# nrclaudio/spVIPES

Hardware: AMD Instinct MI355X
Metric: cells/sec/training-step (2-group PoE VAE) (higher is better)
Workload: dtype bf16

## Files before the change

### spvipes_amd/csrc/spv_abi.hip

```cpp
#include "../../include/spvipes_hip.h"
#include "spv_common.h"
#include "spv_gemm.h"
#include "spv_fc1.h"
#include "spv_dec_gemm.h"
#include "spv_decoder.h"
#include "spv_dec_expected.h"
#include "spv_dec_sample.h"
#include "spv_dec_sample_stats.h"
#include "spv_dec_expected_stats.h"
#include "spv_de.h"
#include "spv_de_median.h"
#include "spv_count_stats.h"
#include "spv_knn.h"
#include "spv_ot.h"
#include "spv_silhouette.h"
#include "spv_small.h"
#include "spv_poe_n.h"

#include <cstdio>
#include <cstdlib>
#include <cstring>

using namespace spv;

// ... 1721 lines not shown
  return SPV_OK;
}
extern "C" int spv_poe_comp_fwd(const spv_poe_comp_args* a, void* stream) {
  int rc = check_poe_comp(a, "spv_poe_comp_fwd", false);
  if (rc) return rc;
  hipStream_t s = (hipStream_t)stream;
  int Bm = 0;
  for (int g = 0; g < a->ngroups; ++g) Bm = a->B[g] > Bm ? a->B[g] : Bm;
  const int W = 2 * a->n + 1;
  hipLaunchKernelGGL(pn_stats_kernel, dim3(PN_SEG, a->ngroups), dim3(128), 0, s, *a);
  hipLaunchKernelGGL(pn_means_kernel, dim3((a->ncomp * W + 255) / 256, a->ngroups), dim3(256), 0, s, *a);
  hipLaunchKernelGGL(pn_fuse_fwd_kernel, dim3((Bm + 7) / 8, a->ngroups), dim3(256), 0, s, *a);
  return launch_status("spv_poe_comp_fwd");
}
extern "C" int spv_poe_comp_bwd(const spv_poe_comp_args* a, void* stream) {
  int rc = check_poe_comp(a, "spv_poe_comp_bwd", true);
  if (rc) return rc;
  hipStream_t s = (hipStream_t)stream;
  int Bm = 0;
  for (int g = 0; g < a->ngroups; ++g) Bm = a->B[g] > Bm ? a->B[g] : Bm;
  hipLaunchKernelGGL(pn_cell_bwd_kernel, dim3((Bm + 7) / 8, a->ngroups), dim3(256), 0, s, *a);
  hipLaunchKernelGGL(pn_comp_bwd_kernel, dim3(PN_SEG, a->ngroups), dim3(64), 0, s, *a);
  hipLaunchKernelGGL(pn_apply_bwd_kernel, dim3((Bm + 7) / 8, a->ngroups), dim3(256), 0, s, *a);
  return launch_status("spv_poe_comp_bwd");
}

extern "C" int spv_zsplit_fwd(const spv_zsplit_args* a, void* stream) {
  if (!a || a->B <= 0 || a->n_p <= 0 || a->n_s <= 0 || a->ngroups <= 0 || a->ngroups > 2) return fail(SPV_ERR_ARG, "spv_zsplit_fwd: bad shape%s");
  for (int g = 0; g < a->ngroups; ++g) if (!a->priv[g] || !a->poe[g] || !a->zcat[g]) return fail(SPV_ERR_ARG, "spv_zsplit_fwd: null pointer%s");
  const long tot = (long)a->B * (a->n_p + a->n_s);
  bool pack = false, pack_all = true;
  for (int g = 0; g < a->ngroups; ++g) { pack = pack || a->am_hi[g] || a->aps_hi[g]; pack_all = pack_all && a->am_hi[g] && a->aps_hi[g]; }
  if (!pack_all) hipLaunchKernelGGL(zsplit_fwd_kernel, dim3((unsigned)((tot + 255) / 256), a->ngroups), dim3(256), 0, (hipStream_t)stream, *a);
  if (pack) {
    const int kp = a->kslots ? SPV_DEC_KP_WIDE : SPV_DEC_KP, ks = a->kslots ? SPV_DEC_KS_WIDE : SPV_DEC_KS;
    if (a->Bp < a->B || (a->kslots != 0 && a->kslots != 1) || a->n_p + 1 > kp || a->n_s + 1 > ks || a->am_cols < a->n_p + a->n_s + 1 || a->am_cols < 0 ||
        a->ld_am < a->am_col + a->am_cols)
      return fail(SPV_ERR_ARG, "spv_zsplit_fwd: bad operand-image shape%s");
    const long tp = (long)a->Bp * (kp + ks + a->am_cols);
    if (a->kslots) hipLaunchKernelGGL(zsplit_pack_kernel<2>, dim3((unsigned)((tp + 255) / 256), a->ngroups), dim3(256), 0, (hipStream_t)stream, *a);
    else hipLaunchKernelGGL(zsplit_pack_kernel<1>, dim3((unsigned)((tp + 255) / 256), a->ngroups), dim3(256), 0, (hipStream_t)stream, *a);
  }
  return launch_status("spv_zsplit_fwd");
}
extern "C" int spv_zsplit_bwd(const spv_zsplit_args* a, void* stream) {
  if (!a || a->B <= 0 || a->n_p <= 0 || a->n_s <= 0 || a->ngroups <= 0 || a->ngroups > 2) return fail(SPV_ERR_ARG, "spv_zsplit_bwd: bad shape%s");
  for (int g = 0; g < a->ngroups; ++g) if (!a->d_zcat[g] || !a->d_priv[g] || !a->d_poe[g]) return fail(SPV_ERR_ARG, "spv_zsplit_bwd: null pointer%s");
  const long tot = (long)a->B * (a->n_p + a->n_s);
  hipLaunchKernelGGL(zsplit_bwd_kernel, dim3((unsigned)((tot + 255) / 256), a->ngroups), dim3(256), 0, (hipStream_t)stream, *a);
  return launch_status("spv_zsplit_bwd");
}

static int check_fold(const spv_fold_batch* a, const char* who) {
  if (!a || a->nprob <= 0 || a->nprob > SPV_MAXP || a->B <= 0) return fail(SPV_ERR_ARG, "%s: bad batch", who);
  if (a->kslots != 0 && a->kslots != 1) return fail(SPV_ERR_ARG, "%s: kslots must be 0 or 1", who);
  const int kmax = a->kslots ? FOLD_KMAX_WIDE : FOLD_KMAX;
  for (int i = 0; i < a->nprob; ++i) {
    const spv_fold_prob& q = a->p[i];
    if (q.K <= 0 || q.K > kmax || q.G <= 0 || q.Gp < q.G || !q.W || !q.gamma || !q.beta || !q.running_mean || !q.running_var || !q.stat ||
        (a->training && (!q.zsum || !q.zz)))
      return fail(SPV_ERR_ARG, "%s: bad problem (K <= 32, or 64 with kslots = 1; non-null pointers)", who);
  }
  return SPV_OK;
}
extern "C" int spv_bn_fold_fwd(const spv_fold_batch* a, void* stream) {
  int rc = check_fold(a, "spv_bn_fold_fwd");
  if (rc) return rc;
  int gmax = 0;
  for (int i = 0; i < a->nprob; ++i) {
    const spv_fold_prob& q = a->p[i];
    if (!q.img_hi || !q.img_lo || q.slot < q.K + 1 || q.col_off + q.slot > q.ld_img) return fail(SPV_ERR_ARG, "spv_bn_fold_fwd: bad image slot%s");
    if ((q.slot | q.col_off | q.ld_img) % 8 || ((reinterpret_cast<uintptr_t>(q.img_hi) | reinterpret_cast<uintptr_t>(q.img_lo)) & 15))
      return fail(SPV_ERR_ARG, "spv_bn_fold_fwd: slot, col_off, ld_img must be multiples of 8 elements and the images 16-byte aligned%s");
    gmax = q.Gp > gmax ? q.Gp : gmax;
  }
  if (a->kslots) hipLaunchKernelGGL(bn_fold_fwd_kernel<FOLD_KMAX_WIDE>, dim3((gmax + FOLD_FWD_GENES - 1) / FOLD_FWD_GENES, a->nprob), dim3(256), 0, (hipStream_t)stream, *a);
  else hipLaunchKernelGGL(bn_fold_fwd_kernel<FOLD_KMAX>, dim3((gmax + FOLD_FWD_GENES - 1) / FOLD_FWD_GENES, a->nprob), dim3(256), 0, (hipStream_t)stream, *a);
  return launch_status("spv_bn_fold_fwd");
}
extern "C" int spv_bn_fold_bwd(const spv_fold_batch* a, void* stream) {
  int rc = check_fold(a, "spv_bn_fold_bwd");
  if (rc) return rc;
  int gmax = 0;
  for (int i = 0; i < a->nprob; ++i) {
    const spv_fold_prob& q = a->p[i];
    if (!q.dWeff || !q.dW || !q.dgamma || !q.dbeta || q.ld_dw < q.K + 1 || (a->training && (!q.red_part || !q.z || !q.dz)))
      return fail(SPV_ERR_ARG, "spv_bn_fold_bwd: null pointer%s");
    gmax = q.G > gmax ? q.G : gmax;
  }
  hipStream_t s = (hipStream_t)stream;
  if (a->kslots) hipLaunchKernelGGL(bn_fold_bwd_kernel<FOLD_KMAX_WIDE>, dim3((gmax + 255) / 256, a->nprob), dim3(FOLD_BWD_THREADS), 0, s, *a);
  else hipLaunchKernelGGL(bn_fold_bwd_kernel<FOLD_KMAX>, dim3((gmax + 255) / 256, a->nprob), dim3(FOLD_BWD_THREADS), 0, s, *a);
  if (a->training) {
    for (int i = 0; i < a->nprob; ++i) {
      const spv_fold_prob& q = a->p[i];
      if (q.out_priv && (!q.out_poe || q.n_p <= 0 || q.n_s <= 0 || q.zcol < 0 || q.zcol + q.K > q.n_p + q.n_s))
        return fail(SPV_ERR_ARG, "spv_bn_fold_bwd: bad latent-slicing outputs%s");
    }
    if (a->kslots) hipLaunchKernelGGL(zstats_bwd_kernel<FOLD_KMAX_WIDE>, dim3((a->B + 63) / 64, a->nprob), dim3(256), 0, s, *a);
    else hipLaunchKernelGGL(zstats_bwd_kernel<FOLD_KMAX>, dim3((a->B + 63) / 64, a->nprob), dim3(256), 0, s, *a);
  }
  return launch_status("spv_bn_fold_bwd");
}

static int check_trunk(const spv_trunk_batch* a, const char* who) {
  if (!a || a->nprob <= 0 || a->nprob > 2 || a->B <= 0) return fail(SPV_ERR_ARG, "%s: bad batch", who);
  for (int i = 0; i < a->nprob; ++i) {
    const spv_trunk_prob& q = a->p[i];
    if (q.N <= 0 || q.N > 256 || q.K <= 0 || q.K > SPV_TRUNK_KMAX) return fail(SPV_ERR_UNSUPPORTED, "%s: N <= 256 and K <= 48", who);
    if (!q.W || !q.gamma || !q.beta || !q.running_mean || !q.running_var || !q.stat) return fail(SPV_ERR_ARG, "%s: null pointer", who);
    if (a->training && (!q.zsum || !q.zz)) return fail(SPV_ERR_ARG, "%s: training mode needs the z statistics", who);
  }
  return SPV_OK;
}
extern "C" int spv_trunk_fold_fwd(const spv_trunk_batch* a, void* stream) {
  int rc = check_trunk(a, "spv_trunk_fold_fwd");
  if (rc) return rc;
  int nmax = 0;
  for (int i = 0; i < a->nprob; ++i) {
    if (!a->p[i].Wf || !a->p[i].cf) return fail(SPV_ERR_ARG, "spv_trunk_fold_fwd: null output%s");
    nmax = a->p[i].N > nmax ? a->p[i].N : nmax;
  }
  hipLaunchKernelGGL(trunk_fold_fwd_kernel, dim3((nmax + TRUNK_FWD_ROWS - 1) / TRUNK_FWD_ROWS, a->nprob), dim3(1024), 0, (hipStream_t)stream, *a);
  return launch_status("spv_trunk_fold_fwd");
}
extern "C" int spv_trunk_fold_bwd(const spv_trunk_batch* a, void* stream) {
  int rc = check_trunk(a, "spv_trunk_fold_bwd");
  if (rc) return rc;
  for (int i = 0; i < a->nprob; ++i) {
    const spv_trunk_prob& q = a->p[i];
    if (!q.dWf || !q.dcf || !q.dW || !q.dgamma || !q.dbeta) return fail(SPV_ERR_ARG, "spv_trunk_fold_bwd: null pointer%s");
    if (a->training && (!q.dred || !q.z || !q.dz || q.ldz < q.K || q.lddz < q.K)) return fail(SPV_ERR_ARG, "spv_trunk_fold_bwd: z-statistics buffers missing%s");
  }
  hipStream_t s = (hipStream_t)stream;
  int nmax = 0;
  for (int i = 0; i < a->nprob; ++i) nmax = a->p[i].N > nmax ? a->p[i].N : nmax;
  const int nblk = (nmax + TRUNK_BWD_ROWS - 1) / TRUNK_BWD_ROWS;
  hipLaunchKernelGGL(trunk_fold_bwd_kernel, dim3(nblk, a->nprob), dim3(1024), 0, s, *a);
  if (a->training) hipLaunchKernelGGL(trunk_zstats_kernel, dim3((a->B + 63) / 64, a->nprob), dim3(256), 0, s, *a, nblk);
  return launch_status("spv_trunk_fold_bwd");
}

extern "C" int spv_reduce_slabs(const spv_reduce_batch* b, void* stream) {
  if (!b || b->nprob <= 0 || b->nprob > SPV_MAXR) return fail(SPV_ERR_ARG, "spv_reduce_slabs: bad batch%s");
  long blocks = 1;
  for (int i = 0; i < b->nprob; ++i) {
    const spv_reduce_prob& q = b->p[i];
    if (!q.src || !q.dst || q.nslabs <= 0 || q.rows <= 0 || q.cols <= 0 || q.ld_src < q.col_off + q.cols || q.ld_dst < q.cols || q.col_off < 0 ||
        (long)q.rows * q.cols >= (1l << 31))
      return fail(SPV_ERR_ARG, "spv_reduce_slabs: bad problem%s");
    const long t = reduce_blocks_needed(q);
    if (t > blocks) blocks = t;
  }
  if (blocks > 8192) blocks = 8192;
  hipLaunchKernelGGL(reduce_slabs_kernel, dim3((unsigned)blocks, b->nprob), dim3(256), 0, (hipStream_t)stream, *b);
  return launch_status("spv_reduce_slabs");
}

extern "C" int spv_loss_assemble(const float* rec0, const float* rec1, const float* w, const float* const* kl, int32_t nkl, int32_t B,
                                 const float* kl_weight, float* loss, float* rec_sum, float* gkl, void* stream) {
  if (!rec0 || !w || !loss || B <= 0 || nkl < 0 || nkl > 4 || (nkl > 0 && !kl)) return fail(SPV_ERR_ARG, "spv_loss_assemble: bad arguments%s");
  const float* k[4] = {nullptr, nullptr, nullptr, nullptr};
  for (int i = 0; i < nkl; ++i) k[i] = kl[i];
  hipLaunchKernelGGL(loss_assemble_kernel, dim3(1), dim3(1024), 0, (hipStream_t)stream, rec0, rec1, w, k[0], k[1], k[2], k[3], B, kl_weight,
                     loss, rec_sum, gkl);
  return launch_status("spv_loss_assemble");
}

struct Fc1PrepArgs { const float* dh1; const float* h1; int B, N1; bf16_t* img_hi; bf16_t* img_lo; long ld_img; float* part; int nblk; float* db; float* db2; int n_first;
                     float* scale_ws; };

__device__ __forceinline__ float block_max_256(float v, float* s_red) {
#pragma unroll
  for (int off = 32; off > 0; off >>= 1) v = fmaxf(v, __shfl_xor(v, off, 64));
  if ((threadIdx.x & 63) == 0) s_red[threadIdx.x >> 6] = v;
  __syncthreads();
  return fmaxf(fmaxf(s_red[0], s_red[1]), fmaxf(s_red[2], s_red[3]));
}

__device__ __forceinline__ void fc1_bwd_prep_body(const Fc1PrepArgs& a, const int blk, float* s_red) {
  const int r0 = blk * 16;
  const bool half = a.img_lo == nullptr;
  float amax = 0.f;
  for (int col = threadIdx.x; col < (int)a.ld_img; col += 256) {
    float sum = 0.f;
#pragma unroll 4
    for (int r = r0; r < r0 + 16; ++r) {
      const long i = (long)min(r, a.B - 1) * a.N1 + min(col, a.N1 - 1);
      const float hv = a.h1[i], gv = a.dh1[i];
      const float v = (r < a.B && col < a.N1 && hv > 0.f) ? gv : 0.f;
      if (!half) {
        bf16_t hi, lo;
        split_bf16(v, hi, lo);
        a.img_hi[(long)r * a.ld_img + col] = hi;
        a.img_lo[(long)r * a.ld_img + col] = lo;
      }
      amax = fmaxf(amax, fabsf(v));
      sum += v;
    }
    if (col < a.N1) a.part[(long)blk * a.N1 + col] = sum;
  }
  if (half) {
    amax = block_max_256(amax, s_red);
    if (threadIdx.x == 0) a.scale_ws[2 + blk] = amax;
  }
}

__device__ __forceinline__ void fc1_bwd_finish_body(const Fc1PrepArgs& a, const int blk, float* s_red, float (*s_p)[64]) {
  const bool half = a.img_lo == nullptr;
  if (half && blk < a.nblk) {
    float m = 0.f;
    for (int k = threadIdx.x; k < a.nblk; k += 256) m = fmaxf(m, a.scale_ws[2 + k]);
    m = block_max_256(m, s_red);
    float scale, inv;
    pow2_scale_for(m, scale, inv);
    if (blk == 0 && threadIdx.x == 0) { a.scale_ws[0] = scale; a.scale_ws[1] = inv; }
    const int r0 = blk * 16;
    for (int col = threadIdx.x; col < (int)a.ld_img; col += 256) {
#pragma unroll 4
      for (int r = r0; r < r0 + 16; ++r) {
        const long i = (long)min(r, a.B - 1) * a.N1 + min(col, a.N1 - 1);
        const float hv = a.h1[i], gv = a.dh1[i];
        const float v = (r < a.B && col < a.N1 && hv > 0.f) ? gv : 0.f;
        a.img_hi[(long)r * a.ld_img + col] = f2h(v * scale);
      }
    }
  }
  if (blk >= (a.N1 + 63) / 64) return;
  const int tx = threadIdx.x & 63, ty = threadIdx.x >> 6;
  const int col = blk * 64 + tx;
  float v = 0.f;
  if (col < a.N1)
#pragma unroll 8
    for (int k = ty; k < a.nblk; k += 4) v += a.part[(long)k * a.N1 + col];
  s_p[ty][tx] = v;
  __syncthreads();
  if (ty != 0 || col >= a.N1) return;
  v = ((s_p[0][tx] + s_p[1][tx]) + s_p[2][tx]) + s_p[3][tx];
  if (a.db2 != nullptr && col >= a.n_first) a.db2[col - a.n_first] = v;
  else a.db[col] = v;
}

__global__ __launch_bounds__(256) void fc1_bwd_prep_kernel(Fc1PrepArgs a) {
  __shared__ float s_red[4];
  fc1_bwd_prep_body(a, blockIdx.x, s_red);
}
__global__ __launch_bounds__(256) void fc1_bwd_finish_kernel(Fc1PrepArgs a) {
  __shared__ float s_red[4];
  __shared__ float s_p[4][64];
  fc1_bwd_finish_body(a, blockIdx.x, s_red, s_p);
}
__global__ __launch_bounds__(256) void fc1_bwd_prep_pair_kernel(Fc1PrepArgs a0, Fc1PrepArgs a1) {
  __shared__ float s_red[4];
  const Fc1PrepArgs a = blockIdx.y ? a1 : a0;
  if ((int)blockIdx.x >= a.nblk) return;
  fc1_bwd_prep_body(a, blockIdx.x, s_red);
}
__global__ __launch_bounds__(256) void fc1_bwd_finish_pair_kernel(Fc1PrepArgs a0, Fc1PrepArgs a1) {
  __shared__ float s_red[4];
  __shared__ float s_p[4][64];
  const Fc1PrepArgs a = blockIdx.y ? a1 : a0;
  fc1_bwd_finish_body(a, blockIdx.x, s_red, s_p);
}
static int fc1_finish_blocks(const Fc1PrepArgs& a) {
  const int nb_bias = (a.N1 + 63) / 64;
  return (a.img_lo == nullptr && a.nblk > nb_bias) ? a.nblk : nb_bias;
}
static Fc1PrepArgs fc1_prep_args(const float* dh1, const float* h1, int B, int N1, uint16_t* img_hi, uint16_t* img_lo, long ld_img, int Bp, float* part, float* db,
                                 float* db2, int n_first, float* scale_ws) {
  return Fc1PrepArgs{dh1, h1, B, N1, (bf16_t*)img_hi, (bf16_t*)img_lo, ld_img, part, Bp / 16, db, db2, n_first, scale_ws};
}
static Fc1PrepArgs fc1_prep_args(const spv_fc1_bwd_args& a) {
  return fc1_prep_args(a.dh1, a.h1, a.B, a.N1, a.dh_hi, nullptr, a.ld_dh, a.Bp, a.part, a.db, a.db2, a.n_first, a.scale_ws);
}
static void fc1_prep_pair_launch(const spv_fc1_bwd_args& a, const spv_fc1_bwd_args& b, hipStream_t s) {
  const Fc1PrepArgs q0 = fc1_prep_args(a), q1 = fc1_prep_args(b);
  hipLaunchKernelGGL(fc1_bwd_prep_pair_kernel, dim3(max2(q0.nblk, q1.nblk), 2), dim3(256), 0, s, q0, q1);
  hipLaunchKernelGGL(fc1_bwd_finish_pair_kernel, dim3(max2(fc1_finish_blocks(q0), fc1_finish_blocks(q1)), 2), dim3(256), 0, s, q0, q1);
}

extern "C" int spv_enc_fc1_bwd_prep(const float* dh1, const float* h1, int32_t B, int32_t N1, uint16_t* img_hi, uint16_t* img_lo,
                                    int64_t ld_img, int32_t Bp, float* part, float* db, float* db2, int32_t n_first, float* scale_ws, void* stream) {
  if (!dh1 || !h1 || !img_hi || !part || !db) return fail(SPV_ERR_ARG, "spv_enc_fc1_bwd_prep: null pointer%s");
  if (B <= 0 || N1 <= 0 || Bp < B || (Bp % 64) || ld_img < N1) return fail(SPV_ERR_ARG, "spv_enc_fc1_bwd_prep: bad shape (Bp a multiple of 64)%s");
  if (!img_lo && !scale_ws) return fail(SPV_ERR_ARG, "spv_enc_fc1_bwd_prep: the f16 image (img_lo == NULL) needs scale_ws [2 + Bp / 16]%s");
  if (Bp / 16 > 65536) return fail(SPV_ERR_ARG, "spv_enc_fc1_bwd_prep: minibatch too large%s");
  hipStream_t s = (hipStream_t)stream;
  const Fc1PrepArgs a = fc1_prep_args(dh1, h1, B, N1, img_hi, img_lo, ld_img, Bp, part, db, db2, n_first, scale_ws);
  hipLaunchKernelGGL(fc1_bwd_prep_kernel, dim3(a.nblk), dim3(256), 0, s, a);
  hipLaunchKernelGGL(fc1_bwd_finish_kernel, dim3(fc1_finish_blocks(a)), dim3(256), 0, s, a);
  return launch_status("spv_enc_fc1_bwd_prep");
}

static bool fc1_fwd_dma_ok(const spv_fc1_fwd_args& a) {
  return a.x && a.x->X && a.W1_hi && a.bias && a.slabs && a.h1 && a.library && a.xb_all && a.library_all && a.B > 0 && a.G > 0 && a.splits > 0 &&
         spv_enc_fc1_fwd_uses_dma(a.B, a.G, a.N1, a.nsplit, 1, a.ldw, a.ld_xb) && aligned16(a.xb_all, a.W1_hi) &&
         (a.nsplit == 1 || (a.W1_lo && aligned16(a.W1_lo)));
}
static GemmParams fc1_fwd_dma_params(const spv_fc1_fwd_args& a) {
  GemmParams p{};
  p.A = a.xb_all; p.lda = a.ld_xb; p.B = a.W1_hi; p.ldb = a.ldw; p.rows = a.x->rows;
  if (a.nsplit == 3) p.B_lo = a.W1_lo;
  p.n_cells = a.B; p.n_genes = a.G; p.C = a.slabs; p.ldc = a.N1; p.M = a.B; p.N = a.N1; p.K = a.G;
  const int kt = (a.G + F1_BK - 1) / F1_BK;
  p.k_per_split = ((kt + a.splits - 1) / a.splits) * F1_BK;
  p.c_split_row = a.splits;
  return p;
// ... 364 lines not shown
```

### spvipes_amd/csrc/spv_small.h

```cpp
#pragma once
#include "../../include/spvipes_hip.h"
#include "spv_common.h"

namespace spv {


typedef spv_linear_prob LinearProb;
typedef spv_linear_batch LinearBatch;

__device__ __forceinline__ unsigned hash_u32(unsigned long long x) {
  x ^= x >> 33; x *= 0xff51afd7ed558ccdULL; x ^= x >> 33; x *= 0xc4ceb9fe1a85ec53ULL; x ^= x >> 33;
  return (unsigned)x;
}
__device__ __forceinline__ bool dropout_keep(unsigned long long seed, int prob, long idx, float p) {
  const unsigned key = ((unsigned)seed ^ ((unsigned)(seed >> 32) * 0x9E3779B9u)) + (unsigned)(prob + 1) * 0x85EBCA6Bu;
  unsigned x = (unsigned)idx * 747796405u + key;
  x = ((x >> ((x >> 28) + 4u)) ^ x) * 277803737u;
  x ^= x >> 22;
  x = x * 0x2C1B3C6Du + key;
  x ^= x >> 15;
  return (float)(x >> 8) * (1.0f / 16777216.0f) >= p;
}

__device__ __forceinline__ f16v mfma_f32(float x, float w, const f16v& c) { return __builtin_amdgcn_mfma_f32_32x32x2f32(x, w, c, 0, 0, 0); }
// ... 1332 lines not shown

constexpr int TRUNK_FWD_ROWS = 16;
__device__ __forceinline__ float trunk_Cw(const float* s_C, const float* wrow, int K, int l) {
  float t = 0.f;
  const int lc = min(l, K - 1);
#pragma unroll 4
  for (int k = 0; k < K; ++k) t += wrow[k] * s_C[k * K + lc];
  return (l < K) ? t : 0.f;
}
__global__ __launch_bounds__(1024) void trunk_fold_fwd_kernel(TrunkBatch a) {
  const TrunkProb& q = a.p[blockIdx.y];
  __shared__ float s_zbar[TRUNK_KMAX], s_C[TRUNK_KMAX * TRUNK_KMAX], s_wr[TRUNK_FWD_ROWS][64];
  const int K = q.K;
  if (blockIdx.x * TRUNK_FWD_ROWS >= q.N) return;
  const int l = threadIdx.x & 63, wv = threadIdx.x >> 6, j = blockIdx.x * TRUNK_FWD_ROWS + wv;
  const int ji = min(j, q.N - 1);
  const float wl = (l < K) ? q.W[(long)ji * K + l] : 0.f;
  const float bj = q.bias ? q.bias[ji] : 0.f;
  s_wr[wv][l] = wl;
  if (a.training) trunk_stats_to_lds(q, a.B, s_zbar, s_C, 1024);
  __syncthreads();
  if (j >= q.N) return;
  float mean0, var;
  if (a.training) {
    const float t = trunk_Cw(s_C, s_wr[wv], K, l);
    mean0 = wave_sum_all(wl * ((l < K) ? s_zbar[l] : 0.f));
    var = fmaxf(wave_sum_all(wl * t), 0.f);
    if (l == 0) {
      q.running_mean[j] = (1.f - a.momentum) * q.running_mean[j] + a.momentum * (mean0 + bj);
      q.running_var[j] = (1.f - a.momentum) * q.running_var[j] + a.momentum * var * ((float)a.B / fmaxf((float)a.B - 1.f, 1.f));
    }
  } else {
    mean0 = q.running_mean[j] - bj;
    var = q.running_var[j];
  }
  const float inv = q.gamma[j] * rsqrtf(var + a.eps);
  if (l < K) q.Wf[(long)j * K + l] = wl * inv;
  if (l == 0) { q.cf[j] = q.beta[j] - inv * mean0; q.stat[2 * j] = mean0; q.stat[2 * j + 1] = var; }
}

constexpr int TRUNK_BWD_ROWS = 64;
__global__ __launch_bounds__(1024) void trunk_fold_bwd_kernel(TrunkBatch a) {
  const TrunkProb& q = a.p[blockIdx.y];
  __shared__ float s_zbar[TRUNK_KMAX], s_C[TRUNK_KMAX * TRUNK_KMAX], s_w[TRUNK_BWD_ROWS * TRUNK_KMAX], s_dm[TRUNK_BWD_ROWS], s_dv[TRUNK_BWD_ROWS];
  const int K = q.K;
  const int j0 = blockIdx.x * TRUNK_BWD_ROWS;
  if (j0 >= q.N) return;
  if (a.training) trunk_stats_to_lds(q, a.B, s_zbar, s_C, 1024);
  __syncthreads();
  const int l = threadIdx.x & 63, wv = threadIdx.x >> 6;
  for (int pass = 0; pass < TRUNK_BWD_ROWS / 16; ++pass) {
    const int jl = 16 * pass + wv, j = j0 + jl;
    const bool real = j < q.N;
    const int ji = min(j, q.N - 1);
    const float wl = (real && l < K) ? q.W[(long)ji * K + l] : 0.f;
    const float gWl = (real && l < K) ? q.dWf[(long)ji * K + l] : 0.f;
    const float mean0 = q.stat[2 * ji], var = q.stat[2 * ji + 1];
    const float rs = rsqrtf(var + a.eps), gam = q.gamma[ji], inv = gam * rs;
    const float gc = real ? q.dcf[ji] : 0.f;
    const float dinv = wave_sum_all(gWl * wl) - gc * mean0;
    float dmean = 0.f, dvar = 0.f;
    if (real && l == 0) {
      q.dbeta[j] = gc;
      q.dgamma[j] = dinv * rs;
      if (q.dbias) q.dbias[j] = a.training ? 0.f : gc * inv;
    }
    if (a.training) {
      if (l < TRUNK_KMAX) s_w[jl * TRUNK_KMAX + l] = wl;
      const float v = trunk_Cw(s_C, s_w + jl * TRUNK_KMAX, K, l);
      if (real) { dmean = -gc * inv; dvar = dinv * gam * (-0.5f) * rs * rs * rs; }
      if (real && l < K) q.dW[(long)j * K + l] = gWl * inv + dmean * s_zbar[l] + 2.0f * dvar * v;
      if (l == 0) { s_dm[jl] = dmean; s_dv[jl] = dvar; }
    } else if (real && l < K) {
      q.dW[(long)j * K + l] = gWl * inv;
    }
  }
  if (!a.training) return;
  __syncthreads();
  const int lane = l, h = lane >> 5, r = lane & 31;
  if (wv >= 4) return;
  const int tr = wv >> 1, tc = wv & 1;
  if (32 * tr >= K || 32 * tc >= K) return;
  f16v accC, accM;
#pragma unroll
  for (int i = 0; i < 16; ++i) { accC[i] = 0.f; accM[i] = 0.f; }
  const int ca = 32 * tr + r, cb = 32 * tc + r;
  for (int t = 0; t < TRUNK_BWD_ROWS; t += 2) {
    const float wa = (ca < TRUNK_KMAX) ? s_w[(t + h) * TRUNK_KMAX + min(ca, TRUNK_KMAX - 1)] : 0.f;
    const float wb = (cb < TRUNK_KMAX) ? s_w[(t + h) * TRUNK_KMAX + min(cb, TRUNK_KMAX - 1)] : 0.f;
    accC = mfma_f32(s_dv[t + h] * wa, wb, accC);
    if (tr == 0) accM = mfma_f32((r == 0) ? s_dm[t + h] : 0.f, wb, accM);
  }
  float* out = q.dred + (long)blockIdx.x * (K + K * K);
#pragma unroll
  for (int i = 0; i < 16; ++i) {
    const int row = 32 * tr + crow(i, h), col = cb;
    if (row < K && col < K) out[K + row * K + col] = accC[i];
  }
  if (tr == 0 && h == 0 && cb < K) out[cb] = accM[0];
}

constexpr int TRUNK_ZS_KK = (TRUNK_KMAX + 3) / 4;
__global__ __launch_bounds__(256) void trunk_zstats_kernel(TrunkBatch a, int nblk) {
  const TrunkProb& q = a.p[blockIdx.y];
  __shared__ float s_zbar[TRUNK_KMAX], s_dz[TRUNK_KMAX], s_S[TRUNK_KMAX * TRUNK_KMAX], s_z[64 * (TRUNK_KMAX + 1)];
  const int K = q.K, nred = K + K * K;
  const float invB = 1.0f / (float)a.B;
  const int nb = (q.N + TRUNK_BWD_ROWS - 1) / TRUNK_BWD_ROWS;
  auto part4 = [&](int i) {
    float v[4];
#pragma unroll
    for (int u = 0; u < 4; ++u) v[u] = q.dred[(long)min(u, nb - 1) * nred + i];
    float d = v[0];
#pragma unroll
    for (int u = 1; u < 4; ++u) d += (u < nb) ? v[u] : 0.f;
    return d;
  };
  for (int i = threadIdx.x; i < K; i += 256) { s_zbar[i] = q.zsum[i] * invB; s_dz[i] = part4(i) * invB; }
  for (int i = threadIdx.x; i < K * K; i += 256) {
    const int k = i / K, l = i - k * K;
    s_S[i] = (part4(K + i) + part4(K + l * K + k)) * invB;
  }
  const int b0 = blockIdx.x * 64;
  __syncthreads();
  for (int i = threadIdx.x; i < 64 * K; i += 256) {
    const int c = i / K, l = i % K, b = min(b0 + c, a.B - 1);
    s_z[c * (TRUNK_KMAX + 1) + l] = q.z[(long)b * q.ldz + l] - s_zbar[l];
  }
  __syncthreads();
  const int c = threadIdx.x & 63, kg = threadIdx.x >> 6;
  float acc[TRUNK_ZS_KK];
#pragma unroll
  for (int kk = 0; kk < TRUNK_ZS_KK; ++kk) acc[kk] = s_dz[min(kg + 4 * kk, K - 1)];
  for (int l = 0; l < K; ++l) {
    const float zl = s_z[c * (TRUNK_KMAX + 1) + l];
#pragma unroll
    for (int kk = 0; kk < TRUNK_ZS_KK; ++kk) acc[kk] += s_S[min(kg + 4 * kk, K - 1) * K + l] * zl;
  }
  __syncthreads();
#pragma unroll
  for (int kk = 0; kk < TRUNK_ZS_KK; ++kk) {
    const int k = kg + 4 * kk;
    if (k < K) s_z[c * (TRUNK_KMAX + 1) + k] = acc[kk];
  }
  __syncthreads();
  (void)nblk;
  for (int i = threadIdx.x; i < 64 * K; i += 256) {
    const int cc = i / K, k = i % K, b = b0 + cc;
    if (b < a.B) q.dz[(long)b * q.lddz + k] += s_z[cc * (TRUNK_KMAX + 1) + k];
  }
}


__device__ __forceinline__ void reduce_finish(const spv_reduce_prob& q, int r, int c, float v, float alpha) {
  v *= alpha;
  if (q.exp_scale) v *= expf(q.exp_scale[c]);
  float* d = q.dst + (long)r * q.ld_dst + c;
  *d = q.accumulate ? *d + v : v;
}
constexpr int RED_FEW_MAX = 8;
template <int V> struct RedVec { float x[V]; };
template <int V> __device__ __forceinline__ RedVec<V> red_ld(const float* p);
template <> __device__ __forceinline__ RedVec<1> red_ld<1>(const float* p) { RedVec<1> r; r.x[0] = *p; return r; }
template <> __device__ __forceinline__ RedVec<4> red_ld<4>(const float* p) {
  const float4 t = *reinterpret_cast<const float4*>(p);
  RedVec<4> r; r.x[0] = t.x; r.x[1] = t.y; r.x[2] = t.z; r.x[3] = t.w; return r;
}
__device__ __forceinline__ void red_st(float* p, const RedVec<1>& v) { *p = v.x[0]; }
__device__ __forceinline__ void red_st(float* p, const RedVec<4>& v) { *reinterpret_cast<float4*>(p) = make_float4(v.x[0], v.x[1], v.x[2], v.x[3]); }
__host__ __device__ inline bool reduce_vec4(const spv_reduce_prob& q) {
  return !((q.cols | q.col_off) & 3) && !((q.ld_src | q.slab_stride | q.ld_dst) & 3) &&
         !(((unsigned long long)q.src | (unsigned long long)q.dst | (unsigned long long)q.exp_scale) & 15ull);
}
template <int NS>
__device__ __forceinline__ float reduce_ordered_sum(const float (&v)[NS]) {
  float acc = v[0];
#pragma unroll
  for (int k = 1; k < NS; ++k) acc += v[k];
  return acc;
}
template <int NS, int V, bool EXTRA>
__device__ __forceinline__ void reduce_few_slabs(const spv_reduce_prob& q, float alpha) {
  const unsigned cols_v = (unsigned)q.cols / V, total = (unsigned)q.rows * cols_v;
  for (unsigned i = blockIdx.x * 256u + threadIdx.x; i < total; i += gridDim.x * 256u) {
    const unsigned r = i / cols_v, c = (i - r * cols_v) * V;
    const float* s = q.src + (long)r * q.ld_src + q.col_off + c;
    float* d = q.dst + (long)r * q.ld_dst + c;
    RedVec<V> v[NS];
#pragma unroll
    for (int k = 0; k < NS; ++k) v[k] = red_ld<V>(s + (long)k * q.slab_stride);
    RedVec<V> e, prev, out;
    if constexpr (EXTRA) {
      e = red_ld<V>(q.exp_scale ? q.exp_scale + c : g_spv_zero4);
      prev = red_ld<V>(q.accumulate ? d : g_spv_zero4);
    }
#pragma unroll
    for (int j = 0; j < V; ++j) {
      float t[NS];
#pragma unroll
      for (int k = 0; k < NS; ++k) t[k] = v[k].x[j];
      float a = reduce_ordered_sum<NS>(t) * alpha;
      if constexpr (EXTRA) {
        if (q.exp_scale) a *= expf(e.x[j]);
        a = q.accumulate ? prev.x[j] + a : a;
      }
      out.x[j] = a;
    }
    red_st(d, out);
  }
}
template <int V, bool EXTRA>
__device__ __forceinline__ void reduce_few_dispatch(const spv_reduce_prob& q, float alpha) {
  switch (q.nslabs) {
    case 1: reduce_few_slabs<1, V, EXTRA>(q, alpha); break;
    case 2: reduce_few_slabs<2, V, EXTRA>(q, alpha); break;
    case 3: reduce_few_slabs<3, V, EXTRA>(q, alpha); break;
    case 4: reduce_few_slabs<4, V, EXTRA>(q, alpha); break;
    case 5: reduce_few_slabs<5, V, EXTRA>(q, alpha); break;
    case 6: reduce_few_slabs<6, V, EXTRA>(q, alpha); break;
    case 7: reduce_few_slabs<7, V, EXTRA>(q, alpha); break;
    default: reduce_few_slabs<8, V, EXTRA>(q, alpha); break;
  }
}
__host__ __device__ inline long reduce_blocks_needed(const spv_reduce_prob& q) {
  const long total = (long)q.rows * q.cols;
  if (q.nslabs > RED_FEW_MAX) return (total + 63) / 64;
  return reduce_vec4(q) ? (total / 4 + 255) / 256 : (total + 255) / 256;
}
__global__ __launch_bounds__(256) void reduce_slabs_kernel(spv_reduce_batch b) {
  __shared__ float s_part[4][64];
  const spv_reduce_prob& q = b.p[blockIdx.y];
  const long total = (long)q.rows * q.cols;
  const float alpha = *(q.alpha ? q.alpha : &g_spv_one);
  if (q.nslabs <= RED_FEW_MAX) {
    const bool extra = q.exp_scale || q.accumulate;
    if (reduce_vec4(q)) { if (extra) reduce_few_dispatch<4, true>(q, alpha); else reduce_few_dispatch<4, false>(q, alpha); }
    else { if (extra) reduce_few_dispatch<1, true>(q, alpha); else reduce_few_dispatch<1, false>(q, alpha); }
    return;
  }
  const int tx = threadIdx.x & 63, ty = threadIdx.x >> 6;
  for (long base = (long)blockIdx.x * 64; base < total; base += (long)gridDim.x * 64) {
    const long i = base + tx;
    const bool ok = i < total;
    int r = 0, c = 0;
    float acc = 0.f;
    if (ok) {
      r = (int)(i / q.cols); c = (int)(i - (long)r * q.cols);
      const float* s = q.src + (long)r * q.ld_src + q.col_off + c;
#pragma unroll 8
      for (int k = ty; k < q.nslabs; k += 4) acc += s[(long)k * q.slab_stride];
    }
    s_part[ty][tx] = acc;
    __syncthreads();
    if (ty == 0 && ok) reduce_finish(q, r, c, ((s_part[0][tx] + s_part[1][tx]) + s_part[2][tx]) + s_part[3][tx], alpha);
    __syncthreads();
  }
}

__global__ __launch_bounds__(1024) void loss_assemble_kernel(const float* rec0, const float* rec1, const float* w, const float* kl0,
                                                             const float* kl1, const float* kl2, const float* kl3, int B,
                                                             const float* kl_weight, float* loss, float* rec_sum, float* gkl) {
  __shared__ float s_r[1024], s_k[1024];
  const int t = threadIdx.x;
  float ar = 0.f, ak = 0.f;
  const float klw = kl_weight ? *kl_weight : 1.f;
  const float gk = klw / (float)B;
  for (int i = t; i < B; i += 1024) {
    const float wi = w[i];
    ar += wi * rec0[i];
    ar += wi * ld_or_zero(rec1, i);
    float k = 0.f;
    k += ld_or_zero(kl0, i);
    k += ld_or_zero(kl1, i);
    k += ld_or_zero(kl2, i);
    k += ld_or_zero(kl3, i);
    ak += k;
    if (gkl) gkl[i] = gk;
  }
  s_r[t] = ar; s_k[t] = ak;
  __syncthreads();
  for (int o = 512; o > 0; o >>= 1) {
    if (t < o) { s_r[t] += s_r[t + o]; s_k[t] += s_k[t + o]; }
    __syncthreads();
  }
  if (t == 0) {
    if (rec_sum) *rec_sum = s_r[0];
    *loss = s_r[0] + gk * s_k[0];
  }
}

}
```

Measured before the change: 6.637 million.

## Restructure slab reduction with per-thread many-slab streaming and CU-capped grid

Reworks the slab-reduction kernel. Large many-slab reductions now have each thread sum all slabs with batched independent loads and 4 accumulators, replacing the shared-memory 4-way split; small ones keep the old shared-memory path. Few-slab items are unrolled two per thread, the grid is capped at a multiple of the CU count queried once, and each problem uses only the blocks it needs, with surplus blocks exiting early. This aims to cut sync/shared-memory overhead and raise memory-level parallelism, but changes summation order and adds code complexity.

```diff
diff --git a/spvipes_amd/csrc/spv_abi.hip b/spvipes_amd/csrc/spv_abi.hip
--- a/spvipes_amd/csrc/spv_abi.hip
+++ b/spvipes_amd/csrc/spv_abi.hip
@@ -1897,7 +1897,16 @@
     const long t = reduce_blocks_needed(q);
     if (t > blocks) blocks = t;
   }
-  if (blocks > 8192) blocks = 8192;
+  static int n_cu[64];
+  int devi = 0, cus = 0;
+  if (hipGetDevice(&devi) != hipSuccess || devi < 0 || devi >= 64) return fail(SPV_ERR_LAUNCH, "spv_reduce_slabs: no device%s");
+  if (!(cus = n_cu[devi])) {
+    if (hipDeviceGetAttribute(&cus, hipDeviceAttributeMultiprocessorCount, devi) != hipSuccess || cus <= 0)
+      return fail(SPV_ERR_LAUNCH, "spv_reduce_slabs: no CU count%s");
+    n_cu[devi] = cus;
+  }
+  const long cap = (long)cus * RED_BLOCKS_PER_CU;
+  if (blocks > cap) blocks = cap;
   hipLaunchKernelGGL(reduce_slabs_kernel, dim3((unsigned)blocks, b->nprob), dim3(256), 0, (hipStream_t)stream, *b);
   return launch_status("spv_reduce_slabs");
 }
diff --git a/spvipes_amd/csrc/spv_small.h b/spvipes_amd/csrc/spv_small.h
--- a/spvipes_amd/csrc/spv_small.h
+++ b/spvipes_amd/csrc/spv_small.h
@@ -1508,13 +1508,9 @@
 }
 
 
-__device__ __forceinline__ void reduce_finish(const spv_reduce_prob& q, int r, int c, float v, float alpha) {
-  v *= alpha;
-  if (q.exp_scale) v *= expf(q.exp_scale[c]);
-  float* d = q.dst + (long)r * q.ld_dst + c;
-  *d = q.accumulate ? *d + v : v;
-}
 constexpr int RED_FEW_MAX = 8;
+constexpr int RED_BATCH = 8;
+constexpr int RED_BLOCKS_PER_CU = 8;
 template <int V> struct RedVec { float x[V]; };
 template <int V> __device__ __forceinline__ RedVec<V> red_ld(const float* p);
 template <> __device__ __forceinline__ RedVec<1> red_ld<1>(const float* p) { RedVec<1> r; r.x[0] = *p; return r; }
@@ -1528,74 +1524,151 @@
   return !((q.cols | q.col_off) & 3) && !((q.ld_src | q.slab_stride | q.ld_dst) & 3) &&
          !(((unsigned long long)q.src | (unsigned long long)q.dst | (unsigned long long)q.exp_scale) & 15ull);
 }
-template <int NS>
-__device__ __forceinline__ float reduce_ordered_sum(const float (&v)[NS]) {
-  float acc = v[0];
-#pragma unroll
-  for (int k = 1; k < NS; ++k) acc += v[k];
-  return acc;
+__host__ __device__ inline int reduce_items_per_trip(const spv_reduce_prob& q) { return q.nslabs > 4 && reduce_vec4(q) ? 1 : 2; }
+constexpr int RED_SMALL_BELOW = 64;
+__host__ __device__ inline long reduce_stream_blocks(const spv_reduce_prob& q) {
+  const long items = (long)q.rows * (reduce_vec4(q) ? q.cols / 4 : q.cols);
+  const int shift = reduce_items_per_trip(q) == 2 ? 9 : 8;
+  return (items + (1l << shift) - 1) >> shift;
+}
+__host__ __device__ inline bool reduce_small(const spv_reduce_prob& q) { return q.nslabs > RED_FEW_MAX && reduce_stream_blocks(q) < RED_SMALL_BELOW; }
+__host__ __device__ inline long reduce_blocks_needed(const spv_reduce_prob& q) {
+  return reduce_small(q) ? ((long)q.rows * q.cols + 63) >> 6 : reduce_stream_blocks(q);
+}
+template <int V> struct RedItem { const float* s; float* d; unsigned c; bool ok; };
+template <int V>
+__device__ __forceinline__ RedItem<V> red_item(const spv_reduce_prob& q, unsigned i, unsigned i_first, unsigned total, unsigned cols_v) {
+  RedItem<V> it;
+  it.ok = i < total;
+  const unsigned ii = it.ok ? i : i_first, r = ii / cols_v;
+  it.c = (ii - r * cols_v) * V;
+  it.s = q.src + (long)r * q.ld_src + q.col_off + it.c;
+  it.d = q.dst + (long)r * q.ld_dst + it.c;
+  return it;
+}
+template <int V>
+__device__ __forceinline__ void red_ld_extra(const spv_reduce_prob& q, const RedItem<V>& it, RedVec<V>& e, RedVec<V>& prev) {
+  e = red_ld<V>(q.exp_scale ? q.exp_scale + it.c : g_spv_zero4);
+  prev = red_ld<V>(q.accumulate ? it.d : g_spv_zero4);
+}
+template <int V, bool EXTRA>
+__device__ __forceinline__ void red_finish(const spv_reduce_prob& q, const RedItem<V>& it, const RedVec<V>& sum, const RedVec<V>& e, const RedVec<V>& prev, float alpha) {
+#pragma clang fp contract(off)
+  RedVec<V> out;
+#pragma unroll
+  for (int j = 0; j < V; ++j) {
+    float a = sum.x[j] * alpha;
+    if constexpr (EXTRA) {
+      if (q.exp_scale) a *= expf(e.x[j]);
+      a = q.accumulate ? prev.x[j] + a : a;
+    }
+    out.x[j] = a;
+  }
+  if (it.ok) red_st(it.d, out);
 }
 template <int NS, int V, bool EXTRA>
-__device__ __forceinline__ void reduce_few_slabs(const spv_reduce_prob& q, float alpha) {
-  const unsigned cols_v = (unsigned)q.cols / V, total = (unsigned)q.rows * cols_v;
-  for (unsigned i = blockIdx.x * 256u + threadIdx.x; i < total; i += gridDim.x * 256u) {
-    const unsigned r = i / cols_v, c = (i - r * cols_v) * V;
-    const float* s = q.src + (long)r * q.ld_src + q.col_off + c;
-    float* d = q.dst + (long)r * q.ld_dst + c;
-    RedVec<V> v[NS];
-#pragma unroll
-    for (int k = 0; k < NS; ++k) v[k] = red_ld<V>(s + (long)k * q.slab_stride);
-    RedVec<V> e, prev, out;
+__device__ __forceinline__ void reduce_few_slabs(const spv_reduce_prob& q, float alpha, unsigned nblocks) {
+  constexpr int U = V * NS > 16 ? 1 : 2;
+  const unsigned cols_v = (unsigned)q.cols / V, total = (unsigned)q.rows * cols_v, stride = nblocks * 256u;
+  for (unsigned i = blockIdx.x * 256u + threadIdx.x; i < total; i += U * stride) {
+    RedItem<V> it[U];
+    RedVec<V> v[U][NS], e[U], prev[U];
+#pragma unroll
+    for (int u = 0; u < U; ++u) {
+      it[u] = red_item<V>(q, i + u * stride, i, total, cols_v);
+#pragma unroll
+      for (int k = 0; k < NS; ++k) v[u][k] = red_ld<V>(it[u].s + (long)k * q.slab_stride);
+      if constexpr (EXTRA) red_ld_extra<V>(q, it[u], e[u], prev[u]);
+    }
+#pragma unroll
+    for (int u = 0; u < U; ++u) {
+      RedVec<V> acc = v[u][0];
+#pragma unroll
+      for (int k = 1; k < NS; ++k)
+#pragma unroll
+        for (int j = 0; j < V; ++j) acc.x[j] += v[u][k].x[j];
+      red_finish<V, EXTRA>(q, it[u], acc, e[u], prev[u], alpha);
+    }
+  }
+}
+template <int V, bool EXTRA>
+__device__ __forceinline__ void reduce_few_dispatch(const spv_reduce_prob& q, float alpha, unsigned nblocks) {
+  switch (q.nslabs) {
+    case 1: reduce_few_slabs<1, V, EXTRA>(q, alpha, nblocks); break;
+    case 2: reduce_few_slabs<2, V, EXTRA>(q, alpha, nblocks); break;
+    case 3: reduce_few_slabs<3, V, EXTRA>(q, alpha, nblocks); break;
+    case 4: reduce_few_slabs<4, V, EXTRA>(q, alpha, nblocks); break;
+    case 5: reduce_few_slabs<5, V, EXTRA>(q, alpha, nblocks); break;
+    case 6: reduce_few_slabs<6, V, EXTRA>(q, alpha, nblocks); break;
+    case 7: reduce_few_slabs<7, V, EXTRA>(q, alpha, nblocks); break;
+    default: reduce_few_slabs<8, V, EXTRA>(q, alpha, nblocks); break;
+  }
+}
+template <int N, int U, int V>
+__device__ __forceinline__ void red_add_batch(const RedItem<V> (&it)[U], long off, long slab_stride, RedVec<V> (&a)[U][4]) {
+  RedVec<V> v[U][N];
+#pragma unroll
+  for (int u = 0; u < U; ++u)
+#pragma unroll
+    for (int k = 0; k < N; ++k) v[u][k] = red_ld<V>(it[u].s + off + (long)k * slab_stride);
+#pragma unroll
+  for (int u = 0; u < U; ++u)
+#pragma unroll
+    for (int k = 0; k < N; ++k)
+#pragma unroll
+      for (int j = 0; j < V; ++j) a[u][k & 3].x[j] += v[u][k].x[j];
+}
+template <int REM, int V, bool EXTRA>
+__device__ __forceinline__ void reduce_many_slabs(const spv_reduce_prob& q, float alpha, unsigned nblocks) {
+  constexpr int U = V == 4 ? 1 : 2;
+  const unsigned cols_v = (unsigned)q.cols / V, total = (unsigned)q.rows * cols_v, stride = nblocks * 256u;
+  const int nfull = q.nslabs / RED_BATCH;
+  for (unsigned i = blockIdx.x * 256u + threadIdx.x; i < total; i += U * stride) {
+    RedItem<V> it[U];
+    RedVec<V> a[U][4], e[U], prev[U];
+#pragma unroll
+    for (int u = 0; u < U; ++u) {
+      it[u] = red_item<V>(q, i + u * stride, i, total, cols_v);
+#pragma unroll
+      for (int y = 0; y < 4; ++y)
+#pragma unroll
+        for (int j = 0; j < V; ++j) a[u][y].x[j] = 0.f;
+    }
+    long off = 0;
+    for (int b = 0; b < nfull; ++b, off += RED_BATCH * q.slab_stride) red_add_batch<RED_BATCH, U, V>(it, off, q.slab_stride, a);
+    if constexpr (REM > 0) red_add_batch<REM, U, V>(it, off, q.slab_stride, a);
     if constexpr (EXTRA) {
-      e = red_ld<V>(q.exp_scale ? q.exp_scale + c : g_spv_zero4);
-      prev = red_ld<V>(q.accumulate ? d : g_spv_zero4);
-    }
-#pragma unroll
-    for (int j = 0; j < V; ++j) {
-      float t[NS];
-#pragma unroll
-      for (int k = 0; k < NS; ++k) t[k] = v[k].x[j];
-      float a = reduce_ordered_sum<NS>(t) * alpha;
-      if constexpr (EXTRA) {
-        if (q.exp_scale) a *= expf(e.x[j]);
-        a = q.accumulate ? prev.x[j] + a : a;
-      }
-      out.x[j] = a;
-    }
-    red_st(d, out);
+      __builtin_amdgcn_sched_barrier(0);
+#pragma unroll
+      for (int u = 0; u < U; ++u) red_ld_extra<V>(q, it[u], e[u], prev[u]);
+    }
+#pragma unroll
+    for (int u = 0; u < U; ++u) {
+      RedVec<V> sum;
+#pragma unroll
+      for (int j = 0; j < V; ++j) sum.x[j] = ((a[u][0].x[j] + a[u][1].x[j]) + a[u][2].x[j]) + a[u][3].x[j];
+      red_finish<V, EXTRA>(q, it[u], sum, e[u], prev[u], alpha);
+    }
   }
 }
 template <int V, bool EXTRA>
-__device__ __forceinline__ void reduce_few_dispatch(const spv_reduce_prob& q, float alpha) {
-  switch (q.nslabs) {
-    case 1: reduce_few_slabs<1, V, EXTRA>(q, alpha); break;
-    case 2: reduce_few_slabs<2, V, EXTRA>(q, alpha); break;
-    case 3: reduce_few_slabs<3, V, EXTRA>(q, alpha); break;
-    case 4: reduce_few_slabs<4, V, EXTRA>(q, alpha); break;
-    case 5: reduce_few_slabs<5, V, EXTRA>(q, alpha); break;
-    case 6: reduce_few_slabs<6, V, EXTRA>(q, alpha); break;
-    case 7: reduce_few_slabs<7, V, EXTRA>(q, alpha); break;
-    default: reduce_few_slabs<8, V, EXTRA>(q, alpha); break;
-  }
-}
-__host__ __device__ inline long reduce_blocks_needed(const spv_reduce_prob& q) {
+__device__ __forceinline__ void reduce_many_dispatch(const spv_reduce_prob& q, float alpha, unsigned nblocks) {
+  switch (q.nslabs % RED_BATCH) {
+    case 0: reduce_many_slabs<0, V, EXTRA>(q, alpha, nblocks); break;
+    case 1: reduce_many_slabs<1, V, EXTRA>(q, alpha, nblocks); break;
+    case 2: reduce_many_slabs<2, V, EXTRA>(q, alpha, nblocks); break;
+    case 3: reduce_many_slabs<3, V, EXTRA>(q, alpha, nblocks); break;
+    case 4: reduce_many_slabs<4, V, EXTRA>(q, alpha, nblocks); break;
+    case 5: reduce_many_slabs<5, V, EXTRA>(q, alpha, nblocks); break;
+    case 6: reduce_many_slabs<6, V, EXTRA>(q, alpha, nblocks); break;
+    default: reduce_many_slabs<7, V, EXTRA>(q, alpha, nblocks); break;
+  }
+}
+__device__ __forceinline__ void reduce_many_small(const spv_reduce_prob& q, float alpha, unsigned nblocks) {
+  __shared__ float s_part[4][64];
   const long total = (long)q.rows * q.cols;
-  if (q.nslabs > RED_FEW_MAX) return (total + 63) / 64;
-  return reduce_vec4(q) ? (total / 4 + 255) / 256 : (total + 255) / 256;
-}
-__global__ __launch_bounds__(256) void reduce_slabs_kernel(spv_reduce_batch b) {
-  __shared__ float s_part[4][64];
-  const spv_reduce_prob& q = b.p[blockIdx.y];
-  const long total = (long)q.rows * q.cols;
-  const float alpha = *(q.alpha ? q.alpha : &g_spv_one);
-  if (q.nslabs <= RED_FEW_MAX) {
-    const bool extra = q.exp_scale || q.accumulate;
-    if (reduce_vec4(q)) { if (extra) reduce_few_dispatch<4, true>(q, alpha); else reduce_few_dispatch<4, false>(q, alpha); }
-    else { if (extra) reduce_few_dispatch<1, true>(q, alpha); else reduce_few_dispatch<1, false>(q, alpha); }
-    return;
-  }
   const int tx = threadIdx.x & 63, ty = threadIdx.x >> 6;
-  for (long base = (long)blockIdx.x * 64; base < total; base += (long)gridDim.x * 64) {
+  for (long base = (long)blockIdx.x * 64; base < total; base += (long)nblocks * 64) {
     const long i = base + tx;
     const bool ok = i < total;
     int r = 0, c = 0;
@@ -1608,9 +1681,29 @@
     }
     s_part[ty][tx] = acc;
     __syncthreads();
-    if (ty == 0 && ok) reduce_finish(q, r, c, ((s_part[0][tx] + s_part[1][tx]) + s_part[2][tx]) + s_part[3][tx], alpha);
+    if (ty == 0 && ok) {
+      float v = (((s_part[0][tx] + s_part[1][tx]) + s_part[2][tx]) + s_part[3][tx]) * alpha;
+      if (q.exp_scale) v *= expf(q.exp_scale[c]);
+      float* d = q.dst + (long)r * q.ld_dst + c;
+      *d = q.accumulate ? *d + v : v;
+    }
     __syncthreads();
   }
+}
+template <int V, bool EXTRA>
+__device__ __forceinline__ void reduce_dispatch(const spv_reduce_prob& q, float alpha, unsigned nblocks) {
+  if (q.nslabs <= RED_FEW_MAX) reduce_few_dispatch<V, EXTRA>(q, alpha, nblocks); else reduce_many_dispatch<V, EXTRA>(q, alpha, nblocks);
+}
+__global__ __launch_bounds__(256) void reduce_slabs_kernel(spv_reduce_batch b) {
+  const spv_reduce_prob q = b.p[blockIdx.y];
+  const long need = reduce_blocks_needed(q);
+  const unsigned nblocks = need < (long)gridDim.x ? (unsigned)need : gridDim.x;
+  if (blockIdx.x >= nblocks) return;
+  const float alpha = *(q.alpha ? q.alpha : &g_spv_one);
+  const bool extra = q.exp_scale || q.accumulate;
+  if (reduce_small(q)) reduce_many_small(q, alpha, nblocks);
+  else if (reduce_vec4(q)) { if (extra) reduce_dispatch<4, true>(q, alpha, nblocks); else reduce_dispatch<4, false>(q, alpha, nblocks); }
+  else { if (extra) reduce_dispatch<1, true>(q, alpha, nblocks); else reduce_dispatch<1, false>(q, alpha, nblocks); }
 }
 
 __global__ __launch_bounds__(1024) void loss_assemble_kernel(const float* rec0, const float* rec1, const float* w, const float* kl0,
```

New measurement: 6.666 million, median of 5. About the same (+0.4%).
